# bababyVN/medical-image-segmentation-and-classification

Measured on AMD Instinct MI355X. Metric: images/sec (train step) Attention U-Net 256x256 bs=32/GPU, higher is better.
Workload: dtype bf16; 1 GPU; AttentionUNet 256x256 train step (fwd+BCE+bwd+clip+AdamW), bs=32/GPU, NHWC bf16 activations, fp32 master weights; global_batch=32, parallelism=dp1, hip_graph=False, wgrad_side_stream=True, plan_replay=C (mi355_plan_run)

## Files before the change

### include/mi355conv.h

```cpp
#ifndef MI355CONV_H_
#define MI355CONV_H_

#include <stdint.h>

#ifdef __cplusplus
extern "C" {
#endif

typedef struct ihipStream_t* mi355_stream_t;

enum { MI355_F32 = 0, MI355_BF16 = 1, MI355_F16 = 2 };
enum { MI355_OK = 0, MI355_ERR_ARG = -1, MI355_ERR_UNSUPPORTED = -2, MI355_ERR_RUNTIME = -3 };

int mi355_version(void);
const char* mi355_last_error(void);


int mi355_pack_input_nchw(const float* x, void* y, int N, int C, int H, int W, int Cpad, int dtype,
                          mi355_stream_t s);
int mi355_pack_input_im2col3(const float* x, void* y, int N, int C, int H, int W, int dtype, mi355_stream_t s);
int mi355_unpack_output_nchw(const void* x, float* y, int N, int C, int H, int W, int ld, int dtype,
                             mi355_stream_t s);
int mi355_pack_nchw(const float* x, void* y, int N, int C, int H, int W, int ld, int dtype, mi355_stream_t s);

int mi355_pack_conv_weight(const float* w, void* wf, void* wb, int Co, int Ci, int Cip, int KH, int KW,
                           int transposed, int dtype, mi355_stream_t s);

int mi355_pack_conv_weights_batched(const int64_t* table, int n, int fields ,
                                    int dtype, mi355_stream_t s);

int mi355_conv2d_igemm(const void* in, const void* wk, const float* bias, void* out,
                       int N, int Hi, int Wi, int Ci, int ldi,
                       int Ho, int Wo, int Co, int ldo,
                       int KH, int KW, int mul, int kmul, int off, int div, int up,
                       int accumulate, float* stats, int dtype, mi355_stream_t s);
int mi355_conv2d_igemm_variant(int Hi, int Wi, int Ci, int Ho, int Wo, int Co, int KH, int KW, int mul, int kmul, int off,
                               int div, int up, int dtype);
int mi355_conv2d_igemm_variant_n(int N, int Hi, int Wi, int Ci, int Ho, int Wo, int Co, int KH, int KW, int mul, int kmul,
                                 int off, int div, int up, int dtype);
int mi355_conv2d_igemm_dma_tile(int N, int Ho, int Wo, int Ci, int Co);
int mi355_conv2d_igemm_generic_tile(int N, int Ho, int Wo, int Co);
int mi355_conv2d_igemm_stat_rows(int N, int Hi, int Wi, int Ci, int Ho, int Wo, int Co, int KH, int KW,
                                 int mul, int kmul, int off, int div, int up, int dtype);
int mi355_conv2d_igemm_pool2_ok(int N, int Hi, int Wi, int Ci, int Ho, int Wo, int Co, int KH, int KW,
                                int mul, int kmul, int off, int div, int up, int dtype);
const char* mi355_conv2d_igemm_kernel_name(int N, int Hi, int Wi, int Ci, int Ho, int Wo, int Co, int KH, int KW,
                                           int mul, int kmul, int off, int div, int up, int dtype);

int mi355_conv2d_wgrad_splits(int N, int Ho, int Wo, int Ci, int Co, int KH, int KW);
int mi355_conv2d_wgrad_variant(int N, int Ho, int Wo, int KH, int KW, int stride, int pad, int dtype);
const char* mi355_conv2d_wgrad_kernel_name(int N, int Ho, int Wo, int Ci, int Co, int KH, int KW, int stride, int pad, int dtype);
int mi355_conv2d_wgrad(const void* x, const void* dy, float* ws, int splits,
                       int N, int Hi, int Wi, int Ci, int ldx,
                       int Ho, int Wo, int Co, int ldy,
                       int KH, int KW, int stride, int pad, int up, int dtype, mi355_stream_t s);
int mi355_conv2d_wgrad_multi_ok(int N, int Ho, int Wo, int dtype);
int mi355_conv2d_wgrad_multi(const void* x0, const void* dy0, const void* x1, const void* dy1, const void* x2, const void* dy2,
                             const void* x3, const void* dy3, const void* x4, const void* dy4, const void* x5, const void* dy5,
                             int napp, float* ws, int splits, int N, int Hi, int Wi, int Ci, int ldx, int Ho, int Wo, int Co,
                             int ldy, int up, int dtype, mi355_stream_t s);
int mi355_conv2d_wgrad_reduce(const float* ws, int splits, float* dw, int Co, int Ci, int Ci_real,
                              int KH, int KW, int transposed, float beta, mi355_stream_t s);


int mi355_rowreduce_blocks(long long M);
int mi355_bn_stats(const void* x, float* partial, long long M, int C, int ld, int dtype, mi355_stream_t s);
int mi355_bn_finalize(const float* partial, int nblocks, long long M, int C, const float* gamma,
                      const float* beta, float* running_mean, float* running_var, int64_t* nbt,
                      float momentum, float eps, float* scale, float* shift, float* mean, float* invstd,
                      mi355_stream_t s);
int mi355_fold_rows(const float* partial, int rows, int rowlen, float* out, int nsplit, mi355_stream_t s);
int mi355_bn_fold_bias(const float* bias, const float* scale, const float* shift, float* out, int C, mi355_stream_t s);
int mi355_bn_eval_coeffs(const float* gamma, const float* beta, const float* running_mean,
                         const float* running_var, float eps, int C, float* scale, float* shift,
                         mi355_stream_t s);
int mi355_bn_act(const void* x, int ldx, const float* scale, const float* shift,
                 const void* x2, int ldx2, const float* scale2, const float* shift2,
                 const void* res, int ldr, void* y, int ldy, long long M, int C, int act, int dtype,
                 mi355_stream_t s);
int mi355_bn_act_pool2(const void* x, int ldx, const float* scale, const float* shift, void* y, int ldy, void* p, int ldp,
                       int N, int H, int W, int C, int act, int dtype, mi355_stream_t s);
int mi355_bn_act_windows(const void* x, int ldx, const float* scale, const float* shift, const void* res, int ldr, void* y, int ldy,
                         int N, int H, int W, int C, int act, int dtype, mi355_stream_t s);
int mi355_bn_bwd_reduce_rows(long long M);
int mi355_bn_bwd_reduce(const void* dy, int lddy, const void* y, int ldy, const void* x, int ldx,
                        const float* mean, const float* invstd, const float* mscale, const float* mshift,
                        float* partial, long long M, int C, int act, int dtype, mi355_stream_t s);
int mi355_bn_bwd_finalize(const float* partial, int nblocks, int C, float* sums, float* dgamma, float* dbeta,
                          float acc, mi355_stream_t s);
int mi355_bn_bwd_finalize_at(const float* partial, int nblocks, int nq, int q0, int q1, int C, float* sums, float* dgamma,
                             float* dbeta, float acc, mi355_stream_t s);
int mi355_bn_bwd_apply(const void* dy, int lddy, const void* y, int ldy, const void* x, int ldx,
                       const float* gamma, const float* mean, const float* invstd, const float* mscale,
                       const float* mshift, const float* sums, void* dx, int lddx, void* dres, int lddres,
                       void* dpost, int lddpost, int post_acc, float* dbias_partial,
                       long long M, int C, int act, int dtype, mi355_stream_t s);
int mi355_bn_bwd_apply_post4(const void* dy, int lddy, const void* y, int ldy, const void* x, int ldx,
                             const float* gamma, const float* mean, const float* invstd, const float* mscale,
                             const float* mshift, const float* sums, void* dx, int lddx, void* dpost, int lddpost,
                             int post_acc, const void* ex0, const void* ex1, const void* ex2, const void* ex3, int ldex,
                             long long M, int C, int act, int dtype, mi355_stream_t s);
int mi355_bn_bwd_pool2_ok(int H, int W, int C, int dtype);
int mi355_bn_bwd_reduce_pool2_rows(long long M);
int mi355_bn_bwd_reduce_pool2(const void* dy, int lddy, const void* dp, int lddp, const void* x, int ldx, const float* mean,
                              const float* invstd, const float* mscale, const float* mshift, float* partial,
                              int N, int H, int W, int C, int dtype, mi355_stream_t s);
int mi355_bn_bwd_apply_pool2(const void* dy, int lddy, const void* dp, int lddp, const void* x, int ldx, const float* gamma,
                             const float* mean, const float* invstd, const float* mscale, const float* mshift,
                             const float* sums, void* dx, int lddx, int N, int H, int W, int C, int dtype, mi355_stream_t s);
int mi355_colsum_finalize(const float* partial, int nblocks, int stride, int C, float* out, float acc,
                          mi355_stream_t s);
int mi355_colsum(const void* x, int ld, float* partial, long long M, int C, int dtype, mi355_stream_t s);

int mi355_maxpool_fwd(const void* x, int ldx, void* y, int ldy, int N, int H, int W, int C,
                      int k, int stride, int pad, int dtype, mi355_stream_t s);
int mi355_maxpool_bwd(const void* x, int ldx, const void* dy, int lddy, void* dx, int lddx,
                      int N, int H, int W, int C, int k, int stride, int pad, int accumulate, int dtype,
                      mi355_stream_t s);
int mi355_upsample2_bwd(const void* dy, int lddy, void* dx, int lddx, int N, int H, int W, int C,
                        int accumulate, int dtype, mi355_stream_t s);
int mi355_add(const void* a, int lda, const void* b, int ldb, void* y, int ldy, long long M, int C, int dtype,
              mi355_stream_t s);
int mi355_relu_fwd(const void* x, int ldx, void* y, int ldy, long long M, int C, int dtype, mi355_stream_t s);
int mi355_relu_bwd(const void* dy, int lddy, const void* y, int ldy, void* dx, int lddx, long long M, int C,
                   int dtype, mi355_stream_t s);

int mi355_rowdot_fwd(const void* x, int ldx, const float* w, const float* b, float* z, float* partial,
                     long long M, int C, int HW, int K, int dtype, mi355_stream_t s);
// ... 239 lines not shown
```

### medical-image-segmentation-and-classification_amd/csrc/conv3x3_ws.hpp

```cpp
#pragma once
#include <type_traits>

#include "common.hpp"
#include "conv3x3_tile.hpp"

template <int CI_, int TH_> struct WsCfg {
  static constexpr int TH = TH_, TW = 32, BN = 64, CI = CI_, NS = CI_ / 32;
  static constexpr int PWL = 36, PH = TH + 2;
  static constexpr int NPIX = PH * PWL;
  static constexpr int P_INSTR = (NPIX + 15) / 16;
  static constexpr int SLAB_BYTES = P_INSTR * 1024;
  static constexpr int C_PITCH = BN * 2 + 8;
  static constexpr int C_BYTES = TH * TW * C_PITCH;
  static constexpr int LDS_BYTES = NS * SLAB_BYTES + C_BYTES;
};

template <int I> using WsI = std::integral_constant<int, I>;
template <int B, int E, typename F> __device__ __forceinline__ void ws_static_for(F&& f) {
  if constexpr (B < E) {
    f(WsI<B>{});
    ws_static_for<B + 1, E>(f);
  }
}

template <typename T, int CI, int TH_>
__global__ __launch_bounds__(256, 2) void conv3x3_ws_kernel(const ConvArgs a, const int groups) {
  static_assert(sizeof(T) == 2, "bf16 / fp16 only");
  typedef WsCfg<CI, TH_> Cfg;
  constexpr int TH = Cfg::TH, TW = Cfg::TW, BN = Cfg::BN, EPC = 8, BM = TH * TW, NS = Cfg::NS;
  constexpr int PWL = Cfg::PWL, PH = Cfg::PH, NPIX = Cfg::NPIX, PIXB = 64;
  constexpr int P_INSTR = Cfg::P_INSTR, P_IT = (P_INSTR + 3) / 4;
  constexpr int SLAB = Cfg::SLAB_BYTES, ROWB = PWL * PIXB;
  constexpr int C_PITCH = Cfg::C_PITCH;
  constexpr int XB = TW / 16, MB = TH * XB;
  constexpr int FRD = CI == 64 ? 3 : 2;
  extern __shared__ __attribute__((aligned(16))) unsigned char lds[];

  const int tid = threadIdx.x, lane = tid & 63, wave = __builtin_amdgcn_readfirstlane(tid >> 6);
  const int l16 = lane & 15, c4 = lane >> 4;
  const int NT = a.Co / BN, TXN = a.Wo / TW, TYN = a.Ho / TH;
  const int S = a.N * TYN * TXN;
  const int xcd = blockIdx.x & 7, j = blockIdx.x >> 3;
  const int nt = j % NT;
  const int kk = xcd * (groups >> 3) + j / NT;
  const int sp_begin = (int)((long long)kk * S / groups), sp_end = (int)((long long)(kk + 1) * S / groups);
  if (sp_begin >= sp_end) return;
  const int n0 = nt * BN;
  const T* __restrict__ in = reinterpret_cast<const T*>(a.in);
  const T* __restrict__ wk = reinterpret_cast<const T*>(a.wk);
  T* __restrict__ out = reinterpret_cast<T*>(a.out);
  const bool flip = a.kmul < 0;

  bf16x8 wf[NS][9];
  {
    const T* wrow = wk + ((size_t)(n0 + wave * 16 + l16) * 9) * Cfg::CI + c4 * EPC;
#pragma unroll
    for (int s = 0; s < NS; ++s)
#pragma unroll
      for (int tp = 0; tp < 9; ++tp) {
        const int tap = flip ? 8 - tp : tp;
        wf[s][tp] = *reinterpret_cast<const bf16x8*>(wrow + tap * Cfg::CI + s * 32);
      }
  }
  f32x4 bias4 = a.bias ? *reinterpret_cast<const f32x4*>(a.bias + n0 + wave * 16 + 4 * c4) : f32x4{0.f, 0.f, 0.f, 0.f};
#pragma unroll
  for (int s = 0; s < NS; ++s)
#pragma unroll
    for (int tp = 0; tp < 9; ++tp) asm volatile("" : "+v"(wf[s][tp]));
  asm volatile("" : "+v"(bias4));

  const int lrow = lane >> 2, slot = lane & 3;
  unsigned p_rel[P_IT];
#pragma unroll
  for (int i = 0; i < P_IT; ++i) {
    const int piece = min(wave + 4 * i, P_INSTR - 1);
    const int q = piece * 16 + lrow;
    const int py = q / PWL, px = q - py * PWL;
    const int ry = a.up ? (py + 1) >> 1 : py, rx = a.up ? (px + 1) >> 1 : px;
    p_rel[i] = (q < NPIX && px < TW + 2) ? (unsigned)(((ry * a.Wi + rx) * a.ldi + (slot ^ (((q >> 2) & 1) << 1)) * EPC) * 2) : DMA_PAD;
  }
  const unsigned lds0 = lds_addr(lds);

  int fa[3];
#pragma unroll
  for (int pw = 0; pw < 3; ++pw) {
    const int x = l16 + pw;
    fa[pw] = x * PIXB + ((c4 ^ (((x >> 2) & 1) << 1)) << 4);
  }

  f32x4 acc[MB];
  T* pend = nullptr;
  bool has_pend = false;
  constexpr int NSTORE = BM * (BN / EPC) / 256;
  constexpr int NSTORE_POOL = (BM / 4) * (BN / EPC) / 256;
  static_assert(NSTORE == TH && NSTORE_POOL * 256 == (BM / 4) * (BN / EPC), "store counts the counted waits rely on");
  const size_t row_stride = (size_t)a.Wo * a.ldo;
  const unsigned char* const cst_rd = lds + NS * Cfg::SLAB_BYTES + (tid >> 3) * C_PITCH + (tid & 7) * 16;
  auto store_pending = [&](int it) __attribute__((always_inline)) {
    const Vec16<T> v = *reinterpret_cast<const Vec16<T>*>(cst_rd + it * TW * C_PITCH);
#ifdef WS64_T_NOSTORE
    if (v.v[0] == (T)12345.f)
#endif
    st16<T>(pend + it * row_stride, v);
  };
#ifdef WS64_SKEW
  if (blockIdx.x >= (gridDim.x >> 1)) {
#pragma unroll 1
    for (int i = 0; i < WS64_SKEW; ++i) __builtin_amdgcn_s_sleep(32);
  }
#endif
  f32x2 wsm[2] = {f32x2{0.f, 0.f}, f32x2{0.f, 0.f}}, wsq[2] = {f32x2{0.f, 0.f}, f32x2{0.f, 0.f}};
  auto tile_of = [&](int sp, int& n, int& ty, int& tx) __attribute__((always_inline)) {
#ifdef WS_ROW_ORDER
    tx = sp % TXN; sp /= TXN;
    ty = sp % TYN;
    n = sp / TYN;
#else
    ty = sp % TYN; sp /= TYN;
    tx = sp % TXN;
    n = sp / TXN;
#endif
  };
  for (int sp = sp_begin; sp < sp_end; ++sp) {
    int n, ty, tx;
    tile_of(sp, n, ty, tx);
    const int y0 = ty * TH, x0 = tx * TW;
    auto patch_of = [&](int sp2, bufdesc_t& desc, unsigned (&off)[P_IT]) __attribute__((always_inline)) {
      int n2, ty2, tx2;
      tile_of(sp2, n2, ty2, tx2);
      const int yy0 = ty2 * TH - 1, xx0 = tx2 * TW - 1;
      const long long org = ((long long)n2 * a.Hi * a.Wi + (long long)(yy0 >> a.up) * a.Wi + (xx0 >> a.up)) * a.ldi;
      desc = make_buf(in + org);
#pragma unroll
      for (int i = 0; i < P_IT; ++i) {
        const int q = min(wave + 4 * i, P_INSTR - 1) * 16 + lrow;
        const int py = q / PWL, px = q - py * PWL;
        const bool ok = (unsigned)(yy0 + py) < (unsigned)a.Hlog && (unsigned)(xx0 + px) < (unsigned)a.Wlog;
        off[i] = ok ? p_rel[i] : DMA_PAD;
      }
    };
    auto issue_piece = [&](const bufdesc_t& desc, const unsigned (&off)[P_IT], int slab, int i) __attribute__((always_inline)) {
      const int piece = min(wave + 4 * i, P_INSTR - 1);
#ifdef WS64_T_NODMA
      if (sp != sp_begin) return;
#endif
      dma16_buf(desc, off[i], (unsigned)slab * 64u, lds0 + slab * SLAB + piece * 1024);
    };
    const bool first = sp == sp_begin;
    if (first) {
      bufdesc_t desc_cur;
      unsigned off_cur[P_IT];
      patch_of(sp, desc_cur, off_cur);
#pragma unroll
      for (int s2 = 0; s2 < NS; ++s2)
#pragma unroll
        for (int i = 0; i < P_IT; ++i) issue_piece(desc_cur, off_cur, s2, i);
      wait_vmcnt<0>();
      __builtin_amdgcn_s_barrier();
    }
    bufdesc_t desc_nxt = make_buf(in, false);
    unsigned off_nxt[P_IT];
    const bool has_next = sp + 1 < sp_end;
    if (has_next) patch_of(sp + 1, desc_nxt, off_nxt);
    else {
#pragma unroll
      for (int i = 0; i < P_IT; ++i) off_nxt[i] = DMA_PAD;
    }

    auto slab_phase = [&](auto slab_tag) __attribute__((always_inline)) {
      constexpr int s = decltype(slab_tag)::value;
      const unsigned char* pa = lds + s * SLAB;
      bf16x8 fr[FRD][XB];
      auto rd = [&](auto v_tag) __attribute__((always_inline)) {
        constexpr int v = decltype(v_tag)::value;
        constexpr int pw = v / PH, pr = v % PH;
#ifdef WS_T_NOSHIFTREAD
        if constexpr (pw > 0) return;
#endif
#pragma unroll
        for (int xb = 0; xb < XB; ++xb)
          fr[v % FRD][xb] = *reinterpret_cast<const bf16x8*>(pa + ((fa[pw] ^ ((pr & 1) << 5)) + pr * ROWB + xb * 16 * PIXB));
      };
      ws_static_for<0, FRD - 1>([&](auto v_tag) __attribute__((always_inline)) { rd(v_tag); });
      ws_static_for<0, 3 * PH>([&](auto v_tag) __attribute__((always_inline)) {
        constexpr int v = decltype(v_tag)::value;
        constexpr int pw = v / PH, pr = v % PH;
        if constexpr (v + FRD - 1 < 3 * PH) rd(WsI<v + FRD - 1>{});
        constexpr int DV = 3 * PH / P_IT, SV = 3 * PH / (NSTORE + 1);
        if constexpr (s >= 1 && v % DV == 0 && v / DV < P_IT) issue_piece(desc_nxt, off_nxt, s - 1, v / DV);
        if constexpr (s == 0 && v % SV == 1 && v / SV < NSTORE) {
          if (has_pend) store_pending(v / SV);
        }
#pragma unroll
        for (int xb = 0; xb < XB; ++xb)
#pragma unroll
          for (int ph = 0; ph < 3; ++ph) {
            const int orow = pr - ph;
            if (orow >= 0 && orow < TH) {
              f32x4& c = acc[orow * XB + xb];
              c = mfma_16x16x32<T>(wf[s][ph * 3 + pw], fr[v % FRD][xb], (s == 0 && pw == 0 && ph == 0) ? bias4 : c);
            }
          }
        __builtin_amdgcn_sched_barrier(0);
      });
    };
    slab_phase(WsI<0>{});
    ws_static_for<1, NS>([&](auto s_tag) __attribute__((always_inline)) {
      if (!first) {
        if (a.pool2) wait_vmcnt<(NS - 2) * P_IT + NSTORE_POOL>(); else wait_vmcnt<(NS - 2) * P_IT + NSTORE>();
      }
      __builtin_amdgcn_s_barrier();
      slab_phase(s_tag);
    });
    wait_vmcnt<(NS - 2) * P_IT>();
    __builtin_amdgcn_s_barrier();

    unsigned char* const cst = lds + NS * SLAB;
    struct alignas(8) Pack4 { T v[4]; };
    auto finish = [&](auto relu_tag, auto stats_tag) __attribute__((always_inline)) {
      constexpr bool RELU = decltype(relu_tag)::value, STATS = decltype(stats_tag)::value;
#pragma unroll
      for (int mb = 0; mb < MB; ++mb) {
        const int row = mb * 16 + l16;
        Pack4 pk;
#pragma unroll
        for (int r = 0; r < 4; ++r) pk.v[r] = from_f32<T>(RELU ? __builtin_amdgcn_fmed3f(acc[mb][r], 0.f, INFINITY) : acc[mb][r]);
        if constexpr (STATS) {
#pragma unroll
          for (int jj = 0; jj < 2; ++jj) {
            const f32x2 v = {to_f32<T>(pk.v[2 * jj]), to_f32<T>(pk.v[2 * jj + 1])};
            wsm[jj] += v;
            wsq[jj] += v * v;
          }
        }
        *reinterpret_cast<Pack4*>(cst + row * C_PITCH + (wave * 16 + 4 * c4) * 2) = pk;
      }
    };
    using Yes = std::true_type;
    using No = std::false_type;
    if (a.stats) {
      if (a.relu) finish(Yes{}, Yes{}); else finish(No{}, Yes{});
    } else {
      if (a.relu) finish(Yes{}, No{}); else finish(No{}, No{});
    }
#pragma unroll
    for (int i = 0; i < P_IT; ++i) issue_piece(desc_nxt, off_nxt, NS - 1, i);
    __builtin_amdgcn_s_waitcnt(0xc07f);
    __builtin_amdgcn_s_barrier();
    constexpr int CPRC = BN / EPC;
    if (a.pool2) {
      const int Ho2 = a.Ho >> 1, Wo2 = a.Wo >> 1;
      for (int id = tid; id < (BM / 4) * CPRC; id += 256) {
        const int g = id / CPRC, c = id - g * CPRC;
        const int gy = g / (TW / 2), gx = g - gy * (TW / 2);
        float sum[EPC];
#pragma unroll
        for (int e = 0; e < EPC; ++e) sum[e] = 0.f;
#pragma unroll
        for (int dy = 0; dy < 2; ++dy)
#pragma unroll
          for (int dx = 0; dx < 2; ++dx) {
            const int row = (2 * gy + dy) * TW + 2 * gx + dx;
            const Vec16<T> v = *reinterpret_cast<const Vec16<T>*>(cst + row * C_PITCH + c * 16);
#pragma unroll
            for (int e = 0; e < EPC; ++e) sum[e] += to_f32<T>(v.v[e]);
          }
        T* p = out + ((size_t)(n * Ho2 + (y0 >> 1) + gy) * Wo2 + (x0 >> 1) + gx) * a.ldo + n0 + c * EPC;
        Vec16<T> v;
        if (a.accumulate) {
          const Vec16<T> o = ld16<T>(p);
#pragma unroll
          for (int e = 0; e < EPC; ++e) v.v[e] = from_f32<T>(sum[e] + to_f32<T>(o.v[e]));
        } else {
#pragma unroll
          for (int e = 0; e < EPC; ++e) v.v[e] = from_f32<T>(sum[e]);
        }
        st16<T>(p, v);
      }
    } else {
      T* const ptile = out + ((size_t)(n * a.Ho + y0) * a.Wo + x0 + (tid >> 3)) * a.ldo + n0 + (tid & 7) * EPC;
      if (a.accumulate) {
        Vec16<T> old[NSTORE];
#pragma unroll
        for (int it = 0; it < NSTORE; ++it) old[it] = ld16<T>(ptile + it * row_stride);
#pragma unroll
        for (int it = 0; it < NSTORE; ++it) {
          Vec16<T> v = *reinterpret_cast<const Vec16<T>*>(cst_rd + it * TW * C_PITCH);
#pragma unroll
          for (int e = 0; e < EPC; ++e) v.v[e] = from_f32<T>(to_f32<T>(v.v[e]) + to_f32<T>(old[it].v[e]));
          st16<T>(ptile + it * row_stride, v);
        }
      } else {
        pend = ptile;
        has_pend = true;
      }
    }
  }
  if (has_pend) {
#pragma unroll
    for (int it = 0; it < NSTORE; ++it) store_pending(it);
  }
  if (a.stats) {
#pragma unroll
    for (int r = 0; r < 4; ++r) {
      const float s1 = row16_sum(wsm[r >> 1][r & 1]), s2 = row16_sum(wsq[r >> 1][r & 1]);
      if (l16 == 0) {
        float* st = a.stats + (size_t)kk * 2 * a.Co + n0 + wave * 16 + 4 * c4 + r;
        st[0] = s1;
        st[a.Co] = s2;
      }
    }
  }
}

static int ws_tile_rows(int Ci, int Ho, int Wo, int Co) {
  if (Co % 64 != 0 || Wo % 32 != 0) return 0;
  if (Ci == 64 && Ho % 8 == 0) return 8;
  if (Ci == 128 && Ho % 4 == 0) return 4;
  return 0;
}

static int ws_groups(int N, int Ho, int Wo, int Co, int th, int cus) {
  const int NT = Co / 64;
  const int S = N * (Ho / th) * (Wo / 32);
  int groups = (2 * cus / NT) & ~7;
  if (groups > (S & ~7)) groups = S & ~7;
  return groups;
}

template <typename T, int CI, int TH>
static int launch_ws(const ConvArgs& a, hipStream_t s, int cus) {
  const int NT = a.Co / 64;
  const int S = a.N * (a.Ho / TH) * (a.Wo / 32);
  const int groups = ws_groups(a.N, a.Ho, a.Wo, a.Co, TH, cus);
  if (groups < 8) MI355_FAIL(MI355_ERR_ARG, "conv3x3_ws: %d spatial tiles are too few for the persistent kernel", S);
  return launch_with_lds<conv3x3_ws_kernel<T, CI, TH>, WsCfg<CI, TH>::LDS_BYTES>("conv3x3_ws", groups * NT, 256, s, a, groups);
}
```

### medical-image-segmentation-and-classification_amd/csrc/conv_igemm.hip

```cpp
#include "common.hpp"
#include <stdlib.h>

struct ConvArgs {
  const void* in;
  const void* wk;
  const float* bias;
  void* out;
  int N, Hi, Wi, Ci, ldi;
  int Ho, Wo, Co, ldo;
  int KH, KW;
  int mul, kmul, off, dshift, up;
  int accumulate;
  int relu;
  int pool2;
  float* stats;
  int M;
  int HoWo;
  int Hlog, Wlog;
};

template <typename T> struct Frag;
template <> struct Frag<bf16_t> {
  static __device__ __forceinline__ void mma(const uint4& a, const uint4& b, f32x16& c) {
    c = __builtin_amdgcn_mfma_f32_32x32x16_bf16(__builtin_bit_cast(bf16x8, a), __builtin_bit_cast(bf16x8, b), c, 0,
// ... 414 lines not shown
        const int col = wn * WTN + ni * 32 + r32;
        *reinterpret_cast<T*>(lds + row * C_PITCH + col * 2) = from_f32<T>(a.relu ? fmaxf(acc[mi][ni][r] + bcol[ni], 0.f) : acc[mi][ni][r] + bcol[ni]);
      }
  __syncthreads();
  if (a.stats && tid < 2 * BN) {
    const int q = tid / BN, c = tid - q * BN;
    float v = 0.f;
#pragma unroll
    for (int w = 0; w < WM; ++w) v += red[(w * 2 + q) * BN + c];
    a.stats[((size_t)mt * 2 + q) * a.Co + n0 + c] = v;
  }
  constexpr int CPRC = BN / EPC;
  for (int id = tid; id < BM * CPRC; id += 256) {
    const int row = id / CPRC, c = id - row * CPRC;
    const int m = m0 + row;
    if (m < a.M) {
      T* p = out + (size_t)m * a.ldo + n0 + c * EPC;
      Vec16<T> v = *reinterpret_cast<const Vec16<T>*>(lds + row * C_PITCH + c * 16);
      if (a.accumulate) {
        const Vec16<T> o = ld16<T>(p);
#pragma unroll
        for (int e = 0; e < EPC; ++e) v.v[e] = from_f32<T>(to_f32<T>(v.v[e]) + to_f32<T>(o.v[e]));
      }
      st16<T>(p, v);
    }
  }
}

template <auto KERNEL, int BN>
static int launch_tiles(const ConvArgs& a, hipStream_t s) {
  hipLaunchKernelGGL(KERNEL, dim3(ceil_div(a.M, 128) * (a.Co / BN)), dim3(256), 0, s, a);
  MI355_LAUNCH_CHECK();
  return MI355_OK;
}
template <typename T, int BN, int BK, int NS>
static int launch_dma(const ConvArgs& a, hipStream_t s) { return launch_tiles<conv_igemm_dma_kernel<T, BN, BK, NS>, BN>(a, s); }

struct ConvShape { int N, Hi, Wi, Ci, Ho, Wo, Co, KH, KW, mul, kmul, off, div, up, dtype; };

#include "conv3x3_halo.hpp"
#include "conv3x3_halo_pp.hpp"
#include "conv3x3_halo_pp128.hpp"
#include "conv3x3_ws.hpp"
#include "conv1x1_stream.hpp"
#include "conv_gemm256.hpp"

template <typename T, int BK>
static int launch_bn(const ConvArgs& a, hipStream_t s, int bn) {
  switch (bn) {
    case 128: return launch_tiles<conv_igemm_kernel<T, 128, BK>, 128>(a, s);
    case 64: return launch_tiles<conv_igemm_kernel<T, 64, BK>, 64>(a, s);
    default: return launch_tiles<conv_igemm_kernel<T, 32, BK>, 32>(a, s);
  }
}

enum IgemmVariant { IG_GENERIC = 0, IG_DMA, IG_HALO_8x32, IG_HALO_16x16, IG_STREAM1x1, IG_HALO_PP, IG_HALO_PP128, IG_WS64, IG_WS128, IG_GEMM256 };

struct ConvChoice {
  IgemmVariant variant;
  IgemmVariant shape_variant;
  int bn, bk, ns;
  int gemm256;
  int stat_rows;
  bool pool2;
};

static int env_int(const char* name, int dflt) { return getenv(name) ? atoi(getenv(name)) : dflt; }
static int device_cus() {
  static const int cus = [] {
    int dev = 0, n = 0;
    if (hipGetDevice(&dev) != hipSuccess || hipDeviceGetAttribute(&n, hipDeviceAttributeMultiprocessorCount, dev) != hipSuccess || n <= 0) n = 256;
    return n;
  }();
  return cus;
}
struct Switches {
  int force_generic = getenv("MI355_IGEMM_VARIANT") ? atoi(getenv("MI355_IGEMM_VARIANT")) == 0 : 0;
  int halo_pp = env_int("MI355_HALO_PP", 0);
  int pp128 = env_int("MI355_HALO_PP128", 1), pp128_min_ci = env_int("MI355_HALO_PP128_MINCI", 256);
  int pp128_fill = env_int("MI355_PP128_FILL", 80);
  int ws64 = env_int("MI355_WS64", 1), ws128 = env_int("MI355_WS128", 1);
  long long ws_min_tiles = getenv("MI355_WS64_MIN_TILES") ? atoll(getenv("MI355_WS64_MIN_TILES")) : 4ll * device_cus();
  int ws128_tile_mult = env_int("MI355_WS128_TILE_MULT", 6);
  int gemm256 = env_int("MI355_GEMM256", 1);
  long long gemm256_min_tiles = getenv("MI355_GEMM256_MIN_TILES") ? atoll(getenv("MI355_GEMM256_MIN_TILES")) : 128;
  int dma_smallgrid = env_int("MI355_DMA_SMALLGRID", 1);
};
static const Switches& switches() { static const Switches sw{}; return sw; }

static bool halo_family(IgemmVariant v) {
  return v == IG_HALO_8x32 || v == IG_HALO_16x16 || v == IG_HALO_PP || v == IG_HALO_PP128 || v == IG_WS64 || v == IG_WS128;
}
static bool image_fits_descriptor(int Hi, int Wi, int ldi, int esz) { return (long long)Hi * Wi * ldi * esz < (1ll << 31); }

static int small_grid_tile_n(long long M, int Co, bool to32) {
  const long long rows = (M + 127) / 128;
  int bn = Co % 128 == 0 ? 128 : (Co % 64 == 0 ? 64 : 32);
  if (switches().dma_smallgrid) {
    const int cus = device_cus();
    if (bn == 128 && rows * (Co / 128) * 2 <= cus) bn = 64;
    if (bn == 64 && to32 && rows * (Co / 64) * 2 <= cus) bn = 32;
  }
  return bn;
}

static IgemmVariant shape_variant(const ConvShape& s, const Switches& sw) {
  if (!dtype_is_2byte(s.dtype) || sw.force_generic) return IG_GENERIC;
  const int Hlog = s.up ? 2 * s.Hi : s.Hi, Wlog = s.up ? 2 * s.Wi : s.Wi;
  const bool is3x3s1 = s.KH == 3 && s.KW == 3 && s.mul == 1 && s.div == 1 && s.Ho == Hlog && s.Wo == Wlog &&
                       ((s.kmul == 1 && s.off == -1) || (s.kmul == -1 && s.off == 1 && !s.up));
  if (is3x3s1 && s.Co % 64 == 0) {
    const bool t16x32 = s.Wo % 32 == 0 && s.Ho % 16 == 0;
    if (sw.halo_pp && t16x32) return IG_HALO_PP;
    if (sw.pp128 && s.Co % 128 == 0 && s.Ci % 64 == 0 && s.Ci >= sw.pp128_min_ci && t16x32) return IG_HALO_PP128;
    const int ws_rows = ws_tile_rows(s.Ci, s.Ho, s.Wo, s.Co);
    if (sw.ws64 && ws_rows == 8) return IG_WS64;
    if (sw.ws128 && ws_rows == 4) return IG_WS128;
    if (s.Wo % 32 == 0 && s.Ho % 8 == 0) return IG_HALO_8x32;
    if (s.Wo % 16 == 0 && s.Ho % 16 == 0) return IG_HALO_16x16;
  }
  if (s.KH == 1 && s.KW == 1 && s.mul == 1 && s.div == 1 && !s.up && s.off == 0 && s.Ho == s.Hi && s.Wo == s.Wi && stream1x1_shape(s.Ci, s.Co))
    return IG_STREAM1x1;
  ConvShape whole = s; whole.N = 256;
  if (sw.gemm256 && gemm256_mode(whole)) return IG_GEMM256;
  if (s.Co % 64 != 0 && s.Ci % 64 != 0) return IG_GENERIC;
  return IG_DMA;
}

static ConvChoice choose(const ConvShape& s) {
  const Switches& sw = switches();
  const int cus = device_cus(), N = s.N, Ho = s.Ho, Wo = s.Wo, Co = s.Co;
  const long long M = (long long)N * Ho * Wo;
  ConvChoice c = {};
  IgemmVariant v = c.shape_variant = shape_variant(s, sw);
  if (v == IG_WS64 || v == IG_WS128) {
    const long long S = (long long)N * (Ho / (v == IG_WS64 ? 8 : 4)) * (Wo / 32);
    if (!(S >= 8 && S * (Co / 64) >= sw.ws_min_tiles * (v == IG_WS128 ? sw.ws128_tile_mult : 1)))
      v = Ho % 8 == 0 ? IG_HALO_8x32 : (Ho % 16 == 0 && Wo % 16 == 0 ? IG_HALO_16x16 : IG_DMA);
  } else if (v == IG_HALO_PP128) {
    const long long grid = (long long)N * (Ho / 16) * (Wo / 32) * (Co / 128);
    const long long rounds = (grid + cus - 1) / cus;
    if (grid * 100 < rounds * cus * sw.pp128_fill) v = IG_HALO_8x32;
  } else if (v == IG_GEMM256) {
    c.gemm256 = gemm256_mode(s);
    if (!c.gemm256 || gemm256_tiles(c.gemm256, N, s.Hi, s.Wi, Ho, Wo, Co) < sw.gemm256_min_tiles) v = IG_DMA, c.gemm256 = 0;
  }
  if (halo_family(v) && !image_fits_descriptor(s.Hi, s.Wi, s.Ci, 2)) v = IG_DMA;
  c.variant = v; c.pool2 = halo_family(v);
  const bool k64 = s.Ci % 64 == 0;
  if (!dtype_is_2byte(s.dtype)) {
    c.bn = small_grid_tile_n(M, Co, true), c.bk = 16;
  } else if (v == IG_GENERIC) {
    c.bn = small_grid_tile_n(M, Co, true), c.bk = k64 ? 64 : 32;
  } else if (v == IG_DMA) {
    c.bn = small_grid_tile_n(M, Co, k64);
    c.bk = c.bn == 64 || (c.bn == 128 && !k64) ? 32 : 64;
    c.ns = c.bn == 128 && k64 ? 2 : 3;
  }
  switch (v) {
    case IG_HALO_PP:
    case IG_HALO_PP128: c.stat_rows = N * (Ho / 16) * (Wo / 32); break;
    case IG_WS128: c.stat_rows = ws_groups(N, Ho, Wo, Co, 4, cus); break;
    case IG_WS64: c.stat_rows = ws_groups(N, Ho, Wo, Co, 8, cus); break;
    case IG_HALO_8x32: c.stat_rows = N * (Ho / 8) * (Wo / 32); break;
    case IG_HALO_16x16: c.stat_rows = N * (Ho / 16) * (Wo / 16); break;
    case IG_DMA: c.stat_rows = ceil_div(M, 128); break;
    case IG_STREAM1x1: c.stat_rows = stream1x1_grid(M); break;
    case IG_GEMM256: c.stat_rows = c.gemm256 == 1 ? (int)(M / 256) : 0; break;
    default: break;
  }
  return c;
}

static ConvArgs conv_args(const ConvShape& s) {
  ConvArgs a = {};
  a.N = s.N; a.Hi = s.Hi; a.Wi = s.Wi; a.Ci = s.Ci;
  a.Ho = s.Ho; a.Wo = s.Wo; a.Co = s.Co;
  a.KH = s.KH; a.KW = s.KW; a.mul = s.mul; a.kmul = s.kmul; a.off = s.off;
  a.dshift = s.div == 1 ? 0 : (s.div == 2 ? 1 : 2); a.up = s.up ? 1 : 0;
  a.M = s.N * s.Ho * s.Wo; a.HoWo = s.Ho * s.Wo;
  a.Hlog = s.up ? 2 * s.Hi : s.Hi; a.Wlog = s.up ? 2 * s.Wi : s.Wi;
  return a;
}

enum { IG_NAME_LEN = 64 };
#define IG_KERNEL(LAUNCH, ...)            \
  if (!name) return LAUNCH;               \
  return snprintf(name, IG_NAME_LEN, __VA_ARGS__) < 0 ? MI355_ERR_ARG : MI355_OK
template <typename T>
static int launch_or_name(const ConvChoice& c, const ConvArgs& a, hipStream_t st, char* name) {
  if constexpr (sizeof(T) == 4) {
    IG_KERNEL((launch_bn<T, 16>(a, st, c.bn)), "conv_igemm_kernel<f32,%d,16>", c.bn);
  } else {
    switch (c.variant) {
      case IG_HALO_PP: IG_KERNEL(launch_halo_pp<T>(a, st), "conv3x3_halo_pp_kernel");
      case IG_HALO_PP128: IG_KERNEL(launch_halo_pp128<T>(a, st), "conv3x3_halo_pp128_kernel");
      case IG_WS64: IG_KERNEL((launch_ws<T, 64, 8>(a, st, device_cus())), "conv3x3_ws_kernel<64,8>");
      case IG_WS128: IG_KERNEL((launch_ws<T, 128, 4>(a, st, device_cus())), "conv3x3_ws_kernel<128,4>");
      case IG_HALO_8x32: IG_KERNEL((launch_halo_rw<T, 8, 32>(a, st)), "conv3x3_halo_rw_kernel<8,32>");
      case IG_HALO_16x16: IG_KERNEL((launch_halo_rw<T, 16, 16>(a, st)), "conv3x3_halo_rw_kernel<16,16>");
      case IG_STREAM1x1: IG_KERNEL(launch_stream1x1<T>(a, st), "conv1x1_stream_kernel<%d,%d>", a.Ci, a.Co);
      case IG_GEMM256: IG_KERNEL(launch_gemm256<T>(a, c.gemm256, st), "conv_gemm256_kernel");
      case IG_DMA:
        switch (c.bn * 100 + c.bk) {
          case 12864: IG_KERNEL((launch_dma<T, 128, 64, 2>(a, st)), "conv_igemm_dma_kernel<128,64,2>");
          case 12832: IG_KERNEL((launch_dma<T, 128, 32, 3>(a, st)), "conv_igemm_dma_kernel<128,32,3>");
          case 6432: IG_KERNEL((launch_dma<T, 64, 32, 3>(a, st)), "conv_igemm_dma_kernel<64,32,3>");
          default: IG_KERNEL((launch_dma<T, 32, 64, 3>(a, st)), "conv_igemm_dma_kernel<32,64,3>");
        }
      default:
        IG_KERNEL((c.bk == 64 ? launch_bn<T, 64>(a, st, c.bn) : launch_bn<T, 32>(a, st, c.bn)), "conv_igemm_kernel<bf16,%d,%d>", c.bn, c.bk);
    }
  }
}
#undef IG_KERNEL

#define GEOM_PARAMS int Hi, int Wi, int Ci, int Ho, int Wo, int Co, int KH, int KW, int mul, int kmul, int off, int div, int up, int dtype
#define GEOM_SHAPE(N) ConvShape{N, Hi, Wi, Ci, Ho, Wo, Co, KH, KW, mul, kmul, off, div, up, dtype}
extern "C" int mi355_conv2d_igemm_variant(GEOM_PARAMS) { return (int)choose(GEOM_SHAPE(1)).shape_variant; }
extern "C" int mi355_conv2d_igemm_variant_n(int N, GEOM_PARAMS) { return (int)choose(GEOM_SHAPE(N)).variant; }
extern "C" int mi355_conv2d_igemm_stat_rows(int N, GEOM_PARAMS) { return choose(GEOM_SHAPE(N)).stat_rows; }
extern "C" int mi355_conv2d_igemm_pool2_ok(int N, GEOM_PARAMS) { return choose(GEOM_SHAPE(N)).pool2; }
extern "C" int mi355_conv2d_igemm_dma_tile(int N, int Ho, int Wo, int Ci, int Co) { return small_grid_tile_n((long long)N * Ho * Wo, Co, Ci % 64 == 0); }
extern "C" int mi355_conv2d_igemm_generic_tile(int N, int Ho, int Wo, int Co) { return small_grid_tile_n((long long)N * Ho * Wo, Co, true); }
extern "C" const char* mi355_conv2d_igemm_kernel_name(int N, GEOM_PARAMS) {
  static thread_local char name[IG_NAME_LEN];
  const ConvShape s = GEOM_SHAPE(N); const ConvChoice c = choose(s);
  const int rc = dispatch_dtype(dtype, "conv2d_igemm_kernel_name", [&](auto tag) { return launch_or_name<decltype(tag)>(c, conv_args(s), nullptr, name); });
  return rc == MI355_OK ? name : nullptr;
}

extern "C" int mi355_conv2d_igemm(const void* in, const void* wk, const float* bias, void* out, int N, int Hi, int Wi,
                                  int Ci, int ldi, int Ho, int Wo, int Co, int ldo, int KH, int KW, int mul, int kmul,
                                  int off, int div, int up, int accumulate, float* stats, int dtype, mi355_stream_t s) {
  MI355_CHECK_ARG(in && wk && out, "conv2d_igemm: null pointer");
  MI355_CHECK_ARG(N > 0 && Hi > 0 && Wi > 0 && Ho > 0 && Wo > 0 && KH > 0 && KW > 0, "conv2d_igemm: bad extent");
  MI355_CHECK_ARG(div == 1 || div == 2 || div == 4, "conv2d_igemm: div must be 1, 2 or 4 (got %d)", div);
  MI355_CHECK_ARG(Co % 32 == 0, "conv2d_igemm: Co=%d must be a multiple of 32", Co);
  MI355_CHECK_ARG(ldi >= Ci && ldo >= Co, "conv2d_igemm: channel stride smaller than channel count");
  MI355_CHECK_ARG((long long)N * Ho * Wo < (1ll << 31) && (long long)N * Hi * Wi < (1ll << 31),
                  "conv2d_igemm: pixel count overflows int32");
  MI355_CHECK_ARG(dtype == MI355_BF16 || dtype == MI355_F16 || dtype == MI355_F32, "conv2d_igemm: unknown dtype %d", dtype);
  const int esz = dtype_is_2byte(dtype) ? 2 : 4;
  MI355_CHECK_ARG(((uintptr_t)in % 16) == 0 && ((uintptr_t)wk % 16) == 0 && ((uintptr_t)out % 16) == 0 &&
                      (ldi * esz) % 16 == 0 && (ldo * esz) % 16 == 0,
                  "conv2d_igemm: pointers / channel strides must be 16-byte aligned");
  MI355_CHECK_ARG(Ci % (esz == 2 ? 32 : 16) == 0, "conv2d_igemm: Ci=%d must be a multiple of %d", Ci, esz == 2 ? 32 : 16);
  const ConvShape shape = GEOM_SHAPE(N);
  const ConvChoice c = choose(shape);
  MI355_CHECK_ARG(!halo_family(c.variant) || image_fits_descriptor(Hi, Wi, ldi, esz),
                  "conv2d_igemm: an image of %d x %d pixels at a channel stride of %d is 2 GiB or more: beyond the 32-bit lane offsets of "
                  "the halo kernels' buffer descriptors", Hi, Wi, ldi);
  MI355_CHECK_ARG(!stats || (c.stat_rows > 0 && !(accumulate & 1)),
                  "conv2d_igemm: fused statistics are not available for this shape/dtype (mi355_conv2d_igemm_stat_rows == 0)");
  ConvArgs a = conv_args(shape);
  a.in = in; a.wk = wk; a.bias = bias; a.out = out;
  a.ldi = ldi; a.ldo = ldo;
  a.accumulate = accumulate & 1;
  a.relu = (accumulate >> 1) & 1;
  a.pool2 = (accumulate >> 2) & 1;
  MI355_CHECK_ARG(!a.pool2 || (c.pool2 && !stats),
                  "conv2d_igemm: the 2x2-sum epilogue exists for the halo kernel only (mi355_conv2d_igemm_variant >= 2)");
  a.stats = stats;
  return dispatch_dtype(dtype, "conv2d_igemm", [&](auto tag) { return launch_or_name<decltype(tag)>(c, a, (hipStream_t)s, nullptr); });
}
```

### medical-image-segmentation-and-classification_amd/csrc/dma.hpp

```cpp
#pragma once
#include "common.hpp"

typedef __attribute__((address_space(3))) void lds_void_t;
typedef __attribute__((address_space(1))) const void gl_void_t;
static __device__ uint4 g_zero_page[16];

#ifdef MI355_DMA_DRAIN
template <int N> __device__ __forceinline__ void wait_vmcnt() { asm volatile("s_waitcnt vmcnt(0)" ::: "memory"); }
#elif defined(MI355_T_NOWAIT)
template <int N> __device__ __forceinline__ void wait_vmcnt() { if (N == 0) asm volatile("s_waitcnt vmcnt(0)" ::: "memory"); }
#else
template <int N> __device__ __forceinline__ void wait_vmcnt() { asm volatile("s_waitcnt vmcnt(%0)" ::"i"(N) : "memory"); }
#endif

__device__ __forceinline__ void dma16(const void* gsrc, unsigned lds_base) {
  unsigned keep;
  asm volatile(
      "s_mov_b32 %0, m0\n\t"
      "s_mov_b32 m0, %2\n\t"
      "s_nop 0\n\t"
      "global_load_lds_dwordx4 %1, off\n\t"
      "s_mov_b32 m0, %0"
      : "=&s"(keep)
      : "v"(gsrc), "s"(lds_base)
      : "memory");
}
__device__ __forceinline__ void dma16_sv(const void* sbase, unsigned voff, unsigned lds_base) {
  unsigned keep;
  asm volatile(
      "s_mov_b32 %0, m0\n\t"
      "s_mov_b32 m0, %3\n\t"
      "s_nop 0\n\t"
      "global_load_lds_dwordx4 %1, %2\n\t"
      "s_mov_b32 m0, %0"
      : "=&s"(keep)
      : "v"(voff), "s"(sbase), "s"(lds_base)
      : "memory");
}
#pragma clang diagnostic push
#pragma clang diagnostic ignored "-Winline-asm"
__device__ __forceinline__ void dma16_sv_m0(const void* sbase, unsigned voff, unsigned lds_byte) {
  asm volatile(
      "s_mov_b32 m0, %2\n\t"
      "s_nop 0\n\t"
      "global_load_lds_dwordx4 %0, %1"
      :
      : "v"(voff), "s"(sbase), "s"(lds_byte)
      : "memory", "m0");
}
#pragma clang diagnostic pop
typedef int __attribute__((ext_vector_type(4))) bufdesc_t;
constexpr unsigned DMA_PAD = 0x80000000u;
__device__ __forceinline__ bufdesc_t make_buf(const void* base, bool valid = true) {
  const unsigned long long p = (unsigned long long)base;
  bufdesc_t d;
  d[0] = (int)(unsigned)p;
  d[1] = (int)(unsigned)((p >> 32) & 0xffffu);
  d[2] = valid ? (int)DMA_PAD : 0;
  d[3] = 0x00020000;
  return d;
}
#pragma clang diagnostic push
#pragma clang diagnostic ignored "-Winline-asm"
__device__ __forceinline__ void dma16_buf(bufdesc_t desc, unsigned voff, unsigned soff, unsigned lds_byte) {
  asm volatile(
      "s_mov_b32 m0, %3\n\t"
      "s_nop 0\n\t"
      "buffer_load_dwordx4 %0, %1, %2 offen lds"
      :
      : "v"(voff), "s"(desc), "s"(soff), "s"(lds_byte)
      : "memory", "m0");
}
#pragma clang diagnostic pop
__device__ __forceinline__ unsigned lds_addr(const void* p) {
  return __builtin_amdgcn_readfirstlane((unsigned)(size_t)(const __attribute__((address_space(3))) void*)p);
}
```

Baseline: 2192 images/s.

## Carry overlapping halo rows between vertically adjacent tiles in persistent 3x3 conv

When the next spatial tile of the persistent WS conv kernel is directly below the current one, the two overlapping halo rows are copied from LDS into the next slab instead of being reloaded from global memory. DMA issue then fetches only the new rows, and the vmcnt waits are adjusted for the different per-tile instruction counts. An optional cap on group count is also added, plus a query for how many tiles are carried. The cost is extra LDS reads and writes, more branching and register pressure in the hot loop, and delicate ordering between the copies and the asynchronous loads.

After: 2185 images/s. About the same (-0.3%).

```diff
diff --git a/include/mi355conv.h b/include/mi355conv.h
--- a/include/mi355conv.h
+++ b/include/mi355conv.h
@@ -44,6 +44,8 @@
                                  int mul, int kmul, int off, int div, int up, int dtype);
 int mi355_conv2d_igemm_pool2_ok(int N, int Hi, int Wi, int Ci, int Ho, int Wo, int Co, int KH, int KW,
                                 int mul, int kmul, int off, int div, int up, int dtype);
+int mi355_conv2d_igemm_ws_carried(int N, int Hi, int Wi, int Ci, int Ho, int Wo, int Co, int KH, int KW,
+                                  int mul, int kmul, int off, int div, int up, int dtype);
 const char* mi355_conv2d_igemm_kernel_name(int N, int Hi, int Wi, int Ci, int Ho, int Wo, int Co, int KH, int KW,
                                            int mul, int kmul, int off, int div, int up, int dtype);
 
diff --git a/medical-image-segmentation-and-classification_amd/csrc/conv3x3_ws.hpp b/medical-image-segmentation-and-classification_amd/csrc/conv3x3_ws.hpp
--- a/medical-image-segmentation-and-classification_amd/csrc/conv3x3_ws.hpp
+++ b/medical-image-segmentation-and-classification_amd/csrc/conv3x3_ws.hpp
@@ -10,6 +10,9 @@
   static constexpr int NPIX = PH * PWL;
   static constexpr int P_INSTR = (NPIX + 15) / 16;
   static constexpr int SLAB_BYTES = P_INSTR * 1024;
+  static constexpr int PC_INSTR = TH * PWL / 16;
+  static constexpr int PC_FIRST_COPY = (TH - 2) * PWL / 16;
+  static_assert(TH % 2 == 0 && (TH * PWL) % 16 == 0 && ((TH - 2) * PWL) % 16 == 8 && PC_INSTR - PC_FIRST_COPY == 5, "carry geometry");
   static constexpr int C_PITCH = BN * 2 + 8;
   static constexpr int C_BYTES = TH * TW * C_PITCH;
   static constexpr int LDS_BYTES = NS * SLAB_BYTES + C_BYTES;
@@ -23,7 +26,7 @@
   }
 }
 
-template <typename T, int CI, int TH_>
+template <typename T, int CI, int TH_, bool CARRY>
 __global__ __launch_bounds__(256, 2) void conv3x3_ws_kernel(const ConvArgs a, const int groups) {
   static_assert(sizeof(T) == 2, "bf16 / fp16 only");
   typedef WsCfg<CI, TH_> Cfg;
@@ -31,6 +34,10 @@
   constexpr int PWL = Cfg::PWL, PH = Cfg::PH, NPIX = Cfg::NPIX, PIXB = 64;
   constexpr int P_INSTR = Cfg::P_INSTR, P_IT = (P_INSTR + 3) / 4;
   constexpr int SLAB = Cfg::SLAB_BYTES, ROWB = PWL * PIXB;
+  constexpr int PC_INSTR = Cfg::PC_INSTR, PC_IT = (PC_INSTR + 3) / 4;
+  constexpr int PC_COPY = Cfg::PC_FIRST_COPY, I_COPY = PC_COPY / 4;
+  constexpr int N_COPY = PC_IT - I_COPY;
+  constexpr int CARRY_LDS = 2 * ROWB;
   constexpr int C_PITCH = Cfg::C_PITCH;
   constexpr int XB = TW / 16, MB = TH * XB;
   constexpr int FRD = CI == 64 ? 3 : 2;
@@ -121,51 +128,99 @@
     n = sp / TXN;
 #endif
   };
+  auto piece_of = [&](int w, int i, bool carry) __attribute__((always_inline)) {
+    const int pc = w + 4 * i;
+    return carry ? (pc < PC_INSTR ? pc : pc - 4) : min(pc, P_INSTR - 1);
+  };
+  const unsigned lds_w = __builtin_amdgcn_readfirstlane(lds0 + wave * 1024);
+  const unsigned lds_wl = __builtin_amdgcn_readfirstlane(lds0 + (piece_of(wave, P_IT - 1, false) - 4 * (P_IT - 1)) * 1024);
+  const unsigned lds_wlc = __builtin_amdgcn_readfirstlane(lds0 + (piece_of(wave, PC_IT - 1, true) - 4 * (PC_IT - 1)) * 1024);
+  bool c_cur = false;
+  auto wait_behind = [&](auto na_tag, auto nb_tag, auto extra_tag, bool c_nxt) __attribute__((always_inline)) {
+    constexpr int NA = decltype(na_tag)::value, NB = decltype(nb_tag)::value, EX = decltype(extra_tag)::value;
+    if constexpr (!CARRY) {
+      wait_vmcnt<(NA + NB) * P_IT + EX>();
+    } else {
+      const bool ca = NA > 0 && c_cur, cb = NB > 0 && c_nxt;
+      if (ca) {
+        if (cb) wait_vmcnt<(NA + NB) * PC_IT + EX>(); else wait_vmcnt<NA * PC_IT + NB * P_IT + EX>();
+      } else {
+        if (cb) wait_vmcnt<NA * P_IT + NB * PC_IT + EX>(); else wait_vmcnt<(NA + NB) * P_IT + EX>();
+      }
+    }
+  };
   for (int sp = sp_begin; sp < sp_end; ++sp) {
     int n, ty, tx;
     tile_of(sp, n, ty, tx);
     const int y0 = ty * TH, x0 = tx * TW;
-    auto patch_of = [&](int sp2, bufdesc_t& desc, unsigned (&off)[P_IT]) __attribute__((always_inline)) {
-      int n2, ty2, tx2;
+    auto patch_of = [&](int sp2, bool carry, bufdesc_t& desc, unsigned (&off)[P_IT]) __attribute__((always_inline)) {
+      int n2, ty2, tx2, w = wave;
+      if constexpr (CARRY) asm volatile("" : "+s"(w));
       tile_of(sp2, n2, ty2, tx2);
-      const int yy0 = ty2 * TH - 1, xx0 = tx2 * TW - 1;
+      const int yy0 = ty2 * TH - 1 + (carry ? 2 : 0), xx0 = tx2 * TW - 1;
       const long long org = ((long long)n2 * a.Hi * a.Wi + (long long)(yy0 >> a.up) * a.Wi + (xx0 >> a.up)) * a.ldi;
       desc = make_buf(in + org);
 #pragma unroll
       for (int i = 0; i < P_IT; ++i) {
-        const int q = min(wave + 4 * i, P_INSTR - 1) * 16 + lrow;
+        const int q = piece_of(w, i, carry) * 16 + lrow;
         const int py = q / PWL, px = q - py * PWL;
         const bool ok = (unsigned)(yy0 + py) < (unsigned)a.Hlog && (unsigned)(xx0 + px) < (unsigned)a.Wlog;
-        off[i] = ok ? p_rel[i] : DMA_PAD;
-      }
-    };
-    auto issue_piece = [&](const bufdesc_t& desc, const unsigned (&off)[P_IT], int slab, int i) __attribute__((always_inline)) {
-      const int piece = min(wave + 4 * i, P_INSTR - 1);
+        unsigned rel = p_rel[i];
+        if (CARRY && carry && w + 4 * i >= PC_INSTR) rel = p_rel[i > 0 ? i - 1 : 0];
+        off[i] = ok ? rel : DMA_PAD;
+      }
+    };
+    auto issue_piece = [&](const bufdesc_t& desc, const unsigned (&off)[P_IT], int slab, int i, bool carry) __attribute__((always_inline)) {
 #ifdef WS64_T_NODMA
       if (sp != sp_begin) return;
 #endif
-      dma16_buf(desc, off[i], (unsigned)slab * 64u, lds0 + slab * SLAB + piece * 1024);
+      if (CARRY && carry) {
+        if (i < PC_IT) dma16_buf_at(desc, off[i], (unsigned)slab * 64u, i == PC_IT - 1 ? lds_wlc : lds_w, slab * SLAB + CARRY_LDS + 4096 * i);
+      } else {
+        dma16_buf_at(desc, off[i], (unsigned)slab * 64u, i == P_IT - 1 ? lds_wl : lds_w, slab * SLAB + 4096 * i);
+      }
     };
     const bool first = sp == sp_begin;
     if (first) {
       bufdesc_t desc_cur;
       unsigned off_cur[P_IT];
-      patch_of(sp, desc_cur, off_cur);
+      patch_of(sp, false, desc_cur, off_cur);
 #pragma unroll
       for (int s2 = 0; s2 < NS; ++s2)
 #pragma unroll
-        for (int i = 0; i < P_IT; ++i) issue_piece(desc_cur, off_cur, s2, i);
+        for (int i = 0; i < P_IT; ++i) issue_piece(desc_cur, off_cur, s2, i, false);
       wait_vmcnt<0>();
       __builtin_amdgcn_s_barrier();
     }
     bufdesc_t desc_nxt = make_buf(in, false);
     unsigned off_nxt[P_IT];
     const bool has_next = sp + 1 < sp_end;
-    if (has_next) patch_of(sp + 1, desc_nxt, off_nxt);
+    bool c_nxt = false;
+    if (CARRY && has_next) {
+      int n2, ty2, tx2;
+      tile_of(sp + 1, n2, ty2, tx2);
+      c_nxt = n2 == n && tx2 == tx && ty2 == ty + 1;
+    }
+    if (has_next) patch_of(sp + 1, c_nxt, desc_nxt, off_nxt);
     else {
 #pragma unroll
       for (int i = 0; i < P_IT; ++i) off_nxt[i] = DMA_PAD;
     }
+    static_assert(N_COPY == 2, "two piece slots of a wave reach into rows TH, TH + 1");
+    typedef unsigned u32x4 __attribute__((ext_vector_type(4)));
+    constexpr int CARRY_DST0 = CARRY_LDS + 4096 * I_COPY - TH * ROWB;
+    auto carry_read = [&](int k, int slab) __attribute__((always_inline)) {
+      int l = lane, w = wave;
+      asm volatile("" : "+v"(l), "+s"(w));
+      return *reinterpret_cast<const u32x4*>(lds + max(w * 1024 + l * 16 + CARRY_DST0 + 4096 * k, 0) + (slab * SLAB + TH * ROWB));
+    };
+    auto carry_write = [&](int k, int slab, u32x4 v) __attribute__((always_inline)) {
+      int l = lane, w = wave;
+      asm volatile("" : "+v"(l), "+s"(w));
+      const int pc = w + 4 * (I_COPY + k);
+      if (pc < PC_INSTR && (pc > PC_COPY || (pc == PC_COPY && l >= 32)))
+        *reinterpret_cast<u32x4*>(lds + max(w * 1024 + l * 16 + CARRY_DST0 + 4096 * k, 0) + slab * SLAB) = v;
+    };
 
     auto slab_phase = [&](auto slab_tag) __attribute__((always_inline)) {
       constexpr int s = decltype(slab_tag)::value;
@@ -181,13 +236,26 @@
         for (int xb = 0; xb < XB; ++xb)
           fr[v % FRD][xb] = *reinterpret_cast<const bf16x8*>(pa + ((fa[pw] ^ ((pr & 1) << 5)) + pr * ROWB + xb * 16 * PIXB));
       };
+      u32x4 cp0 = {0, 0, 0, 0}, cp1 = {0, 0, 0, 0};
       ws_static_for<0, FRD - 1>([&](auto v_tag) __attribute__((always_inline)) { rd(v_tag); });
       ws_static_for<0, 3 * PH>([&](auto v_tag) __attribute__((always_inline)) {
         constexpr int v = decltype(v_tag)::value;
         constexpr int pw = v / PH, pr = v % PH;
         if constexpr (v + FRD - 1 < 3 * PH) rd(WsI<v + FRD - 1>{});
         constexpr int DV = 3 * PH / P_IT, SV = 3 * PH / (NSTORE + 1);
-        if constexpr (s >= 1 && v % DV == 0 && v / DV < P_IT) issue_piece(desc_nxt, off_nxt, s - 1, v / DV);
+        constexpr int CR = CI == 64 ? 0 : 4;
+        static_assert(2 < DV * I_COPY && CR + 2 < DV * (I_COPY + 1), "a chunk is written before the pieces that replace its source are issued");
+        if constexpr (CARRY && s >= 1) {
+          if constexpr (v == 0) cp0 = carry_read(0, s - 1);
+          if constexpr (v == CR) cp1 = carry_read(1, s - 1);
+          if constexpr (v == 2) {
+            if (c_nxt) carry_write(0, s - 1, cp0);
+          }
+          if constexpr (v == CR + 2) {
+            if (c_nxt) carry_write(1, s - 1, cp1);
+          }
+        }
+        if constexpr (s >= 1 && v % DV == 0 && v / DV < P_IT) issue_piece(desc_nxt, off_nxt, s - 1, v / DV, c_nxt);
         if constexpr (s == 0 && v % SV == 1 && v / SV < NSTORE) {
           if (has_pend) store_pending(v / SV);
         }
@@ -206,14 +274,18 @@
     };
     slab_phase(WsI<0>{});
     ws_static_for<1, NS>([&](auto s_tag) __attribute__((always_inline)) {
+      constexpr int s = decltype(s_tag)::value;
       if (!first) {
-        if (a.pool2) wait_vmcnt<(NS - 2) * P_IT + NSTORE_POOL>(); else wait_vmcnt<(NS - 2) * P_IT + NSTORE>();
+        if (a.pool2) wait_behind(WsI<NS - 1 - s>{}, WsI<s - 1>{}, WsI<NSTORE_POOL>{}, c_nxt);
+        else wait_behind(WsI<NS - 1 - s>{}, WsI<s - 1>{}, WsI<NSTORE>{}, c_nxt);
       }
       __builtin_amdgcn_s_barrier();
       slab_phase(s_tag);
     });
-    wait_vmcnt<(NS - 2) * P_IT>();
+    wait_behind(WsI<0>{}, WsI<NS - 2>{}, WsI<0>{}, c_nxt);
     __builtin_amdgcn_s_barrier();
+    u32x4 cl0 = {0, 0, 0, 0}, cl1 = {0, 0, 0, 0};
+    if constexpr (CARRY) cl0 = carry_read(0, NS - 1), cl1 = carry_read(1, NS - 1);
 
     unsigned char* const cst = lds + NS * SLAB;
     struct alignas(8) Pack4 { T v[4]; };
@@ -243,8 +315,9 @@
     } else {
       if (a.relu) finish(Yes{}, No{}); else finish(No{}, No{});
     }
-#pragma unroll
-    for (int i = 0; i < P_IT; ++i) issue_piece(desc_nxt, off_nxt, NS - 1, i);
+    if (CARRY && c_nxt) carry_write(0, NS - 1, cl0), carry_write(1, NS - 1, cl1);
+#pragma unroll
+    for (int i = 0; i < P_IT; ++i) issue_piece(desc_nxt, off_nxt, NS - 1, i, c_nxt);
     __builtin_amdgcn_s_waitcnt(0xc07f);
     __builtin_amdgcn_s_barrier();
     constexpr int CPRC = BN / EPC;
@@ -295,6 +368,7 @@
         has_pend = true;
       }
     }
+    c_cur = c_nxt;
   }
   if (has_pend) {
 #pragma unroll
@@ -320,19 +394,30 @@
   return 0;
 }
 
-static int ws_groups(int N, int Ho, int Wo, int Co, int th, int cus) {
+static int ws_groups(int N, int Ho, int Wo, int Co, int th, int cus, int max_groups) {
   const int NT = Co / 64;
   const int S = N * (Ho / th) * (Wo / 32);
   int groups = (2 * cus / NT) & ~7;
   if (groups > (S & ~7)) groups = S & ~7;
+  if (max_groups >= 8 && groups > (max_groups & ~7)) groups = max_groups & ~7;
   return groups;
 }
 
+static long long ws_carried_tiles(int N, int Ho, int Wo, int Co, int th, int groups) {
+  const int TYN = Ho / th;
+  const long long S = (long long)N * TYN * (Wo / 32);
+  long long carried = 0;
+  for (int kk = 0; kk < groups; ++kk)
+    for (long long sp = kk * S / groups + 1; sp < (kk + 1) * S / groups; ++sp) carried += sp % TYN != 0;
+  return carried * (Co / 64);
+}
+
 template <typename T, int CI, int TH>
-static int launch_ws(const ConvArgs& a, hipStream_t s, int cus) {
+static int launch_ws(const ConvArgs& a, hipStream_t s, int cus, int max_groups, bool carry) {
   const int NT = a.Co / 64;
   const int S = a.N * (a.Ho / TH) * (a.Wo / 32);
-  const int groups = ws_groups(a.N, a.Ho, a.Wo, a.Co, TH, cus);
+  const int groups = ws_groups(a.N, a.Ho, a.Wo, a.Co, TH, cus, max_groups);
   if (groups < 8) MI355_FAIL(MI355_ERR_ARG, "conv3x3_ws: %d spatial tiles are too few for the persistent kernel", S);
-  return launch_with_lds<conv3x3_ws_kernel<T, CI, TH>, WsCfg<CI, TH>::LDS_BYTES>("conv3x3_ws", groups * NT, 256, s, a, groups);
-}
+  if (carry) return launch_with_lds<conv3x3_ws_kernel<T, CI, TH, true>, WsCfg<CI, TH>::LDS_BYTES>("conv3x3_ws", groups * NT, 256, s, a, groups);
+  return launch_with_lds<conv3x3_ws_kernel<T, CI, TH, false>, WsCfg<CI, TH>::LDS_BYTES>("conv3x3_ws", groups * NT, 256, s, a, groups);
+}
diff --git a/medical-image-segmentation-and-classification_amd/csrc/conv_igemm.hip b/medical-image-segmentation-and-classification_amd/csrc/conv_igemm.hip
--- a/medical-image-segmentation-and-classification_amd/csrc/conv_igemm.hip
+++ b/medical-image-segmentation-and-classification_amd/csrc/conv_igemm.hip
@@ -520,6 +520,8 @@
   int ws64 = env_int("MI355_WS64", 1), ws128 = env_int("MI355_WS128", 1);
   long long ws_min_tiles = getenv("MI355_WS64_MIN_TILES") ? atoll(getenv("MI355_WS64_MIN_TILES")) : 4ll * device_cus();
   int ws128_tile_mult = env_int("MI355_WS128_TILE_MULT", 6);
+  int ws_carry = env_int("MI355_WS_CARRY", 1);
+  int ws_max_groups = env_int("MI355_WS_MAX_GROUPS", 0);
   int gemm256 = env_int("MI355_GEMM256", 1);
   long long gemm256_min_tiles = getenv("MI355_GEMM256_MIN_TILES") ? atoll(getenv("MI355_GEMM256_MIN_TILES")) : 128;
   int dma_smallgrid = env_int("MI355_DMA_SMALLGRID", 1);
@@ -598,8 +600,8 @@
   switch (v) {
     case IG_HALO_PP:
     case IG_HALO_PP128: c.stat_rows = N * (Ho / 16) * (Wo / 32); break;
-    case IG_WS128: c.stat_rows = ws_groups(N, Ho, Wo, Co, 4, cus); break;
-    case IG_WS64: c.stat_rows = ws_groups(N, Ho, Wo, Co, 8, cus); break;
+    case IG_WS128: c.stat_rows = ws_groups(N, Ho, Wo, Co, 4, cus, sw.ws_max_groups); break;
+    case IG_WS64: c.stat_rows = ws_groups(N, Ho, Wo, Co, 8, cus, sw.ws_max_groups); break;
     case IG_HALO_8x32: c.stat_rows = N * (Ho / 8) * (Wo / 32); break;
     case IG_HALO_16x16: c.stat_rows = N * (Ho / 16) * (Wo / 16); break;
     case IG_DMA: c.stat_rows = ceil_div(M, 128); break;
@@ -633,8 +635,8 @@
     switch (c.variant) {
       case IG_HALO_PP: IG_KERNEL(launch_halo_pp<T>(a, st), "conv3x3_halo_pp_kernel");
       case IG_HALO_PP128: IG_KERNEL(launch_halo_pp128<T>(a, st), "conv3x3_halo_pp128_kernel");
-      case IG_WS64: IG_KERNEL((launch_ws<T, 64, 8>(a, st, device_cus())), "conv3x3_ws_kernel<64,8>");
-      case IG_WS128: IG_KERNEL((launch_ws<T, 128, 4>(a, st, device_cus())), "conv3x3_ws_kernel<128,4>");
+      case IG_WS64: IG_KERNEL((launch_ws<T, 64, 8>(a, st, device_cus(), switches().ws_max_groups, switches().ws_carry != 0)), "conv3x3_ws_kernel<64,8>");
+      case IG_WS128: IG_KERNEL((launch_ws<T, 128, 4>(a, st, device_cus(), switches().ws_max_groups, switches().ws_carry != 0)), "conv3x3_ws_kernel<128,4>");
       case IG_HALO_8x32: IG_KERNEL((launch_halo_rw<T, 8, 32>(a, st)), "conv3x3_halo_rw_kernel<8,32>");
       case IG_HALO_16x16: IG_KERNEL((launch_halo_rw<T, 16, 16>(a, st)), "conv3x3_halo_rw_kernel<16,16>");
       case IG_STREAM1x1: IG_KERNEL(launch_stream1x1<T>(a, st), "conv1x1_stream_kernel<%d,%d>", a.Ci, a.Co);
@@ -659,6 +661,11 @@
 extern "C" int mi355_conv2d_igemm_variant_n(int N, GEOM_PARAMS) { return (int)choose(GEOM_SHAPE(N)).variant; }
 extern "C" int mi355_conv2d_igemm_stat_rows(int N, GEOM_PARAMS) { return choose(GEOM_SHAPE(N)).stat_rows; }
 extern "C" int mi355_conv2d_igemm_pool2_ok(int N, GEOM_PARAMS) { return choose(GEOM_SHAPE(N)).pool2; }
+extern "C" int mi355_conv2d_igemm_ws_carried(int N, GEOM_PARAMS) {
+  const ConvChoice c = choose(GEOM_SHAPE(N));
+  if ((c.variant != IG_WS64 && c.variant != IG_WS128) || !switches().ws_carry) return 0;
+  return (int)ws_carried_tiles(N, Ho, Wo, Co, c.variant == IG_WS64 ? 8 : 4, c.stat_rows);
+}
 extern "C" int mi355_conv2d_igemm_dma_tile(int N, int Ho, int Wo, int Ci, int Co) { return small_grid_tile_n((long long)N * Ho * Wo, Co, Ci % 64 == 0); }
 extern "C" int mi355_conv2d_igemm_generic_tile(int N, int Ho, int Wo, int Co) { return small_grid_tile_n((long long)N * Ho * Wo, Co, true); }
 extern "C" const char* mi355_conv2d_igemm_kernel_name(int N, GEOM_PARAMS) {
diff --git a/medical-image-segmentation-and-classification_amd/csrc/dma.hpp b/medical-image-segmentation-and-classification_amd/csrc/dma.hpp
--- a/medical-image-segmentation-and-classification_amd/csrc/dma.hpp
+++ b/medical-image-segmentation-and-classification_amd/csrc/dma.hpp
@@ -71,6 +71,15 @@
       : "v"(voff), "s"(desc), "s"(soff), "s"(lds_byte)
       : "memory", "m0");
 }
+__device__ __forceinline__ void dma16_buf_at(bufdesc_t desc, unsigned voff, unsigned soff, unsigned lds_base, int lds_imm) {
+  asm volatile(
+      "s_add_u32 m0, %3, %4\n\t"
+      "s_nop 0\n\t"
+      "buffer_load_dwordx4 %0, %1, %2 offen lds"
+      :
+      : "v"(voff), "s"(desc), "s"(soff), "s"(lds_base), "i"(lds_imm)
+      : "memory", "m0", "scc");
+}
 #pragma clang diagnostic pop
 __device__ __forceinline__ unsigned lds_addr(const void* p) {
   return __builtin_amdgcn_readfirstlane((unsigned)(size_t)(const __attribute__((address_space(3))) void*)p);
```
